# adamjorr/kbbq

Hardware: AMD Instinct MI355X
Metric: recalibrated Gbases/sec (higher is better)
Workload: dtype u64

## Files before the change

### kbbq_amd/csrc/engine.hip

```cpp
#include <hip/hip_runtime.h>

#include <algorithm>
#include <climits>
#include <cstdarg>
#include <cstdio>
#include <cstdlib>
#include <cstring>
#include <map>
#include <mutex>
#include <string>
#include <thread>
#include <vector>

#include "../../include/kbbq_engine.h"
#include "abi_internal.h"
#include "correct.h"
#include "correct_wave.h"
#include "device_common.h"
#include "host_model.h"

using namespace kbbq;

static thread_local char g_err[512] = "";
int kbbq_fail(int code, const char *fmt, ...) {
// ... 27 lines not shown
    FiltDev dev() const {
        FiltDev f;
        f.table = reinterpret_cast<ulonglong2 *>(d_table);
        f.patterns = reinterpret_cast<const ulonglong2 *>(d_patterns);
        f.n_blocks = spec.n_blocks;
        const ModMagic mm = make_mod_magic(spec.n_blocks);
        f.mod_magic = mm.m64;
        f.mod_m32 = mm.m32;
        f.salt0 = spec.salt[0];
        f.salt1 = spec.salt[1];
        return f;
    }
};

struct ProfileSlot {
    std::string name;
    uint64_t launches = 0;
    double ms = 0;
};
struct PendingEvent {
    int slot;
    hipEvent_t a, b;
};

constexpr int kNoOverride = INT_MIN;
struct Options {
    bool no_overlap = false;
    bool no_fastpath = false;
    bool lane_walk = false;
    bool no_pass4_pipeline = false;
    int pass2_side = 2;
    bool tally_general = false;
    bool infer_subset = true;
    bool debug_bucket = false;
    int bucket = -1;
    uint64_t bucket_records = 0;
    uint64_t pass4_piece = 0;
    int scan_blocks = -1;
    int walk_blocks = -1;
    int infer_blocks = 0;
    int subset_edge = kNoOverride;
    int subset_pmask = kNoOverride;
};


enum Scratch {
    S_KMER_PREFIX,
    S_HOST_OUT,
    S_HOST_FLAGS,
    S_DRAW0, S_DRAW1,
    S_TAKE1,
    S_READ_INDEX0, S_READ_INDEX1,
    S_TMASK, S_DIRTY, S_LIST, S_ERR, S_PATCH,
    S_OFFCASE_LIST,
    S_WALK_WORDS,
    S_SIDE1,
    S_COUNT = S_SIDE1 + (S_SIDE1 - S_TMASK),
    S_TAKE0 = S_ERR + (S_SIDE1 - S_TMASK),
};
constexpr int per_side(Scratch name, int side) { return name + side * (S_SIDE1 - S_TMASK); }

struct SideCounters { unsigned long long list_len, queries; };
struct Counters {
    SideCounters side0;
    unsigned long long kmer_total;
    unsigned long long infer_fetched;
// ... 71 lines not shown
    bool cur_h2d_recorded = false;
    bool async_call = false;
    uint64_t last_ticket = 0;
    hipStream_t copy = nullptr;
    uint64_t stats[4] = {0, 0, 0, 0};
    std::vector<ProfileSlot> prof;
    std::vector<PendingEvent> pending;
    uint32_t *d_qcum = nullptr, *d_errthr = nullptr;
    uint32_t qcum_len = 0;
    struct Buckets {
        int mode[2] = {-1, -1};
        bool allocated = false;
        uint64_t capacity = 0;
        void *l1 = nullptr, *l2 = nullptr;
        uint32_t *l1_cnt = nullptr, *l2_cnt = nullptr, *tickets = nullptr;
        unsigned long long *direct = nullptr;
        bool pending[2] = {false, false};
        double pending_est[2] = {0, 0};
        double frac_trusted = 0.75;
        double frac_used = 0.75;
        uint64_t bases_since[2] = {0, 0}, inserted_at_flush[2] = {0, 0};
        uint64_t flushes[2] = {0, 0};
        hipStream_t stream[2] = {nullptr, nullptr};
        hipEvent_t ev_flush = nullptr;
        unsigned long long *h_inserted = nullptr;
        hipEvent_t ev_est = nullptr;
        bool est_pending = false, est_known = false;
        uint64_t est_bases = 0, est_prev = 0, cur_bases = 0;
    } bk;
    hipEvent_t ev_infer = nullptr, ev_take[2] = {nullptr, nullptr};
    bool take_pending[2] = {false, false};
    int take_turn = 0;
    size_t attr_lds_tally = 0, attr_lds_recal = 0;
    std::map<const void *, size_t> attr_lds_correct;
};

namespace {

template <typename T> int scratch_buf(kbbq_engine *e, int name, size_t bytes, T **out) {
    if (e->scratch_bytes[name] < bytes) {
        if (e->scratch[name]) {
            HIP_TRY(hipStreamSynchronize(e->stream));
            HIP_TRY(hipStreamSynchronize(e->stream2));
            HIP_TRY(hipFree(e->scratch[name]));
            e->scratch[name] = nullptr;
            e->scratch_bytes[name] = 0;
        }
        const size_t want = bytes + bytes / 8 + 256;
        HIP_TRY(hipMalloc(&e->scratch[name], want));
        e->scratch_bytes[name] = want;
    }
    *out = static_cast<T *>(e->scratch[name]);
    return KBBQ_OK;
}

int run_after(hipStream_t waiter, hipStream_t signaller, hipEvent_t ev) {
    HIP_TRY(hipEventRecord(ev, signaller));
    HIP_TRY(hipStreamWaitEvent(waiter, ev, 0));
    return KBBQ_OK;
}

std::vector<hipEvent_t *> engine_events(kbbq_engine *e) {
    std::vector<hipEvent_t *> v = {&e->ev_main, &e->ev_draw, &e->ev_ins[0], &e->ev_ins[1], &e->ev_side[0], &e->ev_side[1],
                                   &e->bk.ev_flush, &e->bk.ev_est, &e->ev_infer, &e->ev_take[0], &e->ev_take[1]};
    for (kbbq_engine::StageSlot &s : e->slot) v.insert(v.end(), {&s.h2d, &s.d2h, &s.done[0], &s.done[1]});
    return v;
// ... 483 lines not shown

}


extern "C" {

const char *kbbq_last_error(void) { return g_err; }

int kbbq_engine_create(const kbbq_params *params, kbbq_engine **out) {
    if (!params || !out) return fail(KBBQ_EINVAL, "null argument");
    if (params->k < 1 || params->k > KBBQ_MAX_KMER) return fail(KBBQ_ERANGE, "k must be <= %d and > 0", KBBQ_MAX_KMER);
    if (params->n_rg < 1 || params->n_rg > 65535) return fail(KBBQ_EINVAL, "n_rg must be in 1..65535");
    if (params->max_read_len < 1 || params->max_read_len > KBBQ_MAX_READ_LEN)
        return fail(KBBQ_ERANGE, "max_read_len must be in 1..%d", KBBQ_MAX_READ_LEN);
    int ndev = 0;
    if (hipGetDeviceCount(&ndev) != hipSuccess || ndev == 0) return fail(KBBQ_ENODEV, "no HIP device visible");
    if (params->device < 0 || params->device >= ndev) return fail(KBBQ_ENODEV, "device %d of %d", params->device, ndev);
    DeviceGuard create_guard(params->device);
    HIP_TRY(create_guard.err);
    kbbq_engine *e = new kbbq_engine;
    e->p = *params;
    {
        Options &o = e->opt;
        auto env_set = [](const char *name) { const char *v = getenv(name); return v && *v; };
        auto env_int = [](const char *name, int dflt) { const char *v = getenv(name); return v && *v ? atoi(v) : dflt; };
        const int fl = params->flags;
        o.no_overlap = (fl & KBBQ_F_NO_OVERLAP) || env_set("KBBQ_NO_OVERLAP");
        o.no_fastpath = (fl & KBBQ_F_NO_FASTPATH) || env_set("KBBQ_NO_FASTPATH");
        o.lane_walk = (fl & KBBQ_F_LANE_WALK) || (getenv("KBBQ_CORRECT") && !strcmp(getenv("KBBQ_CORRECT"), "lane"));
        o.no_pass4_pipeline = (fl & KBBQ_F_NO_PASS4_PIPELINE) || env_set("KBBQ_NO_PASS4_PIPELINE");
        o.pass2_side = (fl & KBBQ_F_PASS2_INORDER) ? 0 : env_int("KBBQ_PASS2_SIDE", o.pass2_side);
        o.tally_general = env_set("KBBQ_TALLY_GENERAL");
        o.infer_subset = env_int("KBBQ_INFER_SUBSET", 1) != 0;
        o.debug_bucket = env_set("KBBQ_DEBUG_BUCKET");
        o.bucket = (fl & KBBQ_F_BUCKET_ON) ? 1 : (fl & KBBQ_F_BUCKET_OFF) ? 0 : env_set("KBBQ_BUCKET") ? (env_int("KBBQ_BUCKET", 0) != 0 ? 1 : 0) : -1;
        o.bucket_records = env_u64("KBBQ_BUCKET_RECORDS", 0);
        o.pass4_piece = env_u64("KBBQ_PASS4_PIECE", 0);
        o.scan_blocks = env_int("KBBQ_SCAN_BLOCKS", o.scan_blocks);
        o.walk_blocks = env_int("KBBQ_WALK_BLOCKS", o.walk_blocks);
        o.infer_blocks = env_int("KBBQ_INFER_BLOCKS", o.infer_blocks);
        o.subset_edge = env_int("KBBQ_SUBSET_EDGE", o.subset_edge);
        o.subset_pmask = env_int("KBBQ_SUBSET_PMASK", o.subset_pmask);
    }
    e->K.k = params->k;
    e->K.shift = 2u * (unsigned)(params->k - 1);
    e->K.mask = params->k < 32 ? ((1ULL << (2 * params->k)) - 1) : ~0ULL;
    e->K.nmask_bits = params->k < 32 ? ((1u << params->k) - 1) : 0xFFFFFFFFu;
    const double fprs[2] = {params->fpr_sampled, params->fpr_trusted};
    for (int w = 0; w < 2; ++w) {
        if (!make_filter_spec(params->approx_kmers, fprs[w], params->bloom_seed, e->filt[w].spec)) {
            delete e;
            return fail(KBBQ_EINVAL, "Error: Invalid bloom filter parameters. Adjust parameters and try again.");
        }
    }
    hipError_t he = hipStreamCreateWithFlags(&e->stream, hipStreamNonBlocking);
    if (he == hipSuccess) he = hipStreamCreateWithFlags(&e->stream2, hipStreamNonBlocking);
    if (he == hipSuccess) he = hipStreamCreateWithFlags(&e->copy, hipStreamNonBlocking);
    for (hipEvent_t *ev : engine_events(e))
        if (he == hipSuccess) he = hipEventCreateWithFlags(ev, hipEventDisableTiming);
    if (he == hipSuccess) he = hipHostMalloc((void **)&e->bk.h_inserted, 64, hipHostMallocDefault);
    if (he != hipSuccess) { kbbq_engine_destroy(e); return fail(KBBQ_EIO, "hipStreamCreate: %s", hipGetErrorString(he)); }
#define CREATE_TRY(expr)                                                                           \
    do {                                                                                           \
        hipError_t _e = (expr);                                                                    \
        if (_e != hipSuccess) {                                                                    \
            int code = _e == hipErrorOutOfMemory ? KBBQ_ENOMEM : KBBQ_EIO;                         \
// ... 104 lines not shown
    for (int w = 0; w < 2; ++w) { e->bk.pending[w] = false; e->bk.pending_est[w] = 0; e->bk.bases_since[w] = 0; e->bk.inserted_at_flush[w] = 0; e->bk.flushes[w] = 0; }
    e->thresholds_set = false;
    e->dq_set = false;
    memset(e->stats, 0, sizeof e->stats);
    return sync_engine(e);
}

int kbbq_engine_sync(kbbq_engine *e) {
    ENGINE_DEVICE(e);
    return settle(e);
}

void *kbbq_engine_stream(kbbq_engine *e) { return e ? (void *)e->stream : nullptr; }

int kbbq_engine_dims(kbbq_engine *e, uint64_t *n_rg, uint64_t *n_cycle) {
    if (!e) return fail(KBBQ_EINVAL, "null engine");
    if (n_rg) *n_rg = (uint64_t)e->p.n_rg;
    if (n_cycle) *n_cycle = (uint64_t)e->p.max_read_len;
    return KBBQ_OK;
}

int kbbq_engine_tune(kbbq_engine *e, const char *name, uint64_t value) {
    if (!e || !name) return fail(KBBQ_EINVAL, "null argument");
    if (!strcmp(name, "bucket_records")) {
        if (e->bk.allocated) return fail(KBBQ_ESTATE, "the record buffers are allocated already");
        e->opt.bucket_records = value;
    } else if (!strcmp(name, "pass4_piece")) {
        e->opt.pass4_piece = value;
    } else if (!strcmp(name, "scan_blocks") || !strcmp(name, "walk_blocks") || !strcmp(name, "infer_blocks")) {
        if (value > 17) return fail(KBBQ_EINVAL, "%s: 0 (as many as fit) to 16 workgroups per CU, 17 = default", name);
        (name[0] == 's' ? e->opt.scan_blocks : name[0] == 'w' ? e->opt.walk_blocks : e->opt.infer_blocks) = value == 17 ? (name[0] == 'i' ? 0 : -1) : (int)value;
    } else if (!strcmp(name, "infer_subset")) {
        e->opt.infer_subset = value != 0;
    } else if (!strcmp(name, "pass2_side") || !strcmp(name, "no_overlap")) {
        ENGINE_DEVICE(e);
        int rc = settle(e);
        if (rc) return rc;
        if (name[0] == 'p' && value > 2) return fail(KBBQ_EINVAL, "pass2_side: 0, 1 or 2");
        if (name[0] == 'p') e->opt.pass2_side = (int)value; else e->opt.no_overlap = value != 0;
        e->bk.stream[0] = e->bk.stream[1] = nullptr;
    } else {
        return fail(KBBQ_EINVAL, "unknown knob '%s'", name);
    }
    return KBBQ_OK;
}

int kbbq_filter_info_get(kbbq_engine *e, int which, kbbq_filter_info *out) {
    ENGINE_DEVICE(e);
    if (!out || which < 0 || which > 1) return fail(KBBQ_EINVAL, "bad argument");
    int rc = settle(e);
    if (rc) return rc;
    const FilterSpec &s = e->filt[which].spec;
    memset(out, 0, sizeof *out);
    out->bits = s.bits;
    out->bits_unblocked = s.bits_unblocked;
    out->n_blocks = s.n_blocks;
    out->table_bytes = e->filt[which].table_bytes();
    out->random_seed = s.random_seed;
    out->n_hash = s.n_hash;
    out->n_salt = s.n_salt;
    for (uint32_t i = 0; i < s.n_salt; ++i) out->salt[i] = s.salt[i];
    HIP_TRY(hipMemcpy(&out->inserted, e->filt[which].d_inserted, 8, hipMemcpyDeviceToHost));
    return KBBQ_OK;
}

void *kbbq_filter_device_table(kbbq_engine *e, int which) {
// ... 817 lines not shown
    hipLaunchKernelGGL(k_read_index, dim3((unsigned)((R.n_reads + 255) / 256)), dim3(256), 0, stream, R.offsets, R.n_reads, d);
    HIP_TRY(hipGetLastError());
    *index = d;
    return KBBQ_OK;
}

static int run_tally(kbbq_engine *e, const Pass3 &c, const ReadsDev &R, const uint32_t *err_bits, const uint32_t *patch, int max_len) {
    const hipStream_t stream = c.stream;
    HistDev H;
    H.cycle = e->d_hist;
    H.dinuc = e->d_hist + e->hist_cycle_words;
    H.n_rg = e->p.n_rg;
    H.n_cycle = e->p.max_read_len;
    const int n_rg = R.rg ? e->p.n_rg : 1;
    const int ccap = std::min(((max_len + 31) / 32) * 32, 192);
    if (!e->qpresent_known) {
        hipLaunchKernelGGL(k_qpresence, dim3(1024), dim3(256), 0, stream, R.qual, R.n_bases, e->d_qpresent);
        HIP_TRY(hipGetLastError());
        HIP_TRY(hipMemcpyAsync(e->qpresent, e->d_qpresent, 32, hipMemcpyDeviceToHost, stream));
        HIP_TRY(hipStreamSynchronize(stream));
    }
    const int n_windows = (max_len + ccap - 1) / ccap;
    const bool direct_cycles = n_windows > kTallyMaxWindows;
    const size_t per_slot = (direct_cycles ? 0 : (size_t)8 * ccap) + 128;
    TallyPlan P;
    plan_tally_slots(P, e->qpresent, (int)((152 * 1024 - 512) / per_slot), n_rg);
    P.direct_cycles = direct_cycles ? 1 : 0;
    const size_t per_rg = (size_t)P.n_slots * per_slot;
    const size_t budget = (size_t)n_rg * per_rg <= 70 * 1024 ? 70 * 1024 : 140 * 1024;
    const int per_launch = (int)std::max<size_t>(1, std::min<size_t>((size_t)n_rg, budget / per_rg));
    const size_t lds = (size_t)per_launch * per_rg + 4 + 256 + 4;
    if (lds > e->attr_lds_tally) {
        HIP_TRY(hipFuncSetAttribute((const void *)k_tally, hipFuncAttributeMaxDynamicSharedMemorySize, (int)lds));
        HIP_TRY(hipFuncSetAttribute((const void *)k_tally_uniform<true>, hipFuncAttributeMaxDynamicSharedMemorySize, (int)lds));
        HIP_TRY(hipFuncSetAttribute((const void *)k_tally_uniform<false>, hipFuncAttributeMaxDynamicSharedMemorySize, (int)lds));
        e->attr_lds_tally = lds;
    }
    const uint64_t groups = (R.n_bases + 15) / 16;
    const int blocks = (int)std::min<uint64_t>((groups + 1023) / 1024, lds <= 76 * 1024 ? 512 : 256);
    const int vec_ok = ((uintptr_t)R.qual & 15) == 0;
    const uint32_t *read_index;
    int rc = build_read_index(e, R, c.stream_no, stream, &read_index);
    if (rc) return rc;
    const uint32_t *present = nullptr;
    if (n_rg > per_launch) {
        uint32_t *pr = e->d_rg_present[c.stream_no];
        HIP_TRY(hipMemsetAsync(pr, 0, (((size_t)e->p.n_rg + 31) / 32) * 4, stream));
        hipLaunchKernelGGL(k_rg_presence, dim3((unsigned)((R.n_reads + 255) / 256)), dim3(256), 0, stream, R.rg, R.n_reads, (uint32_t)e->p.n_rg, pr);
        present = pr;
    }
    if (!e->opt.tally_general && !R.offsets && n_rg == 1 && n_windows == 1 && R.read_len >= 16 && (int)R.read_len <= ccap && R.n_bases < (1ULL << 32) && vec_ok &&
        e->p.n_rg == 1) {
        const unsigned long long inv_len = ~0ULL / R.read_len + 1;
        Timed t(e, "k_tally", stream);
        if (P.identity) hipLaunchKernelGGL(k_tally_uniform<false>, dim3(blocks), dim3(1024), lds, stream, R, H, err_bits, patch, ccap, 6, inv_len, P);
        else hipLaunchKernelGGL(k_tally_uniform<true>, dim3(blocks), dim3(1024), lds, stream, R, H, err_bits, patch, ccap, 6, inv_len, P);
        HIP_TRY(hipGetLastError());
        return KBBQ_OK;
    }
    Timed t(e, "k_tally", stream);
    for (int g = 0; g < n_rg; g += per_launch)
        for (int w = 0; w < (direct_cycles ? 1 : n_windows); ++w) {
            P.rg_base = g;
            P.n_rgs = std::min(per_launch, n_rg - g);
            P.cbase = w * ccap;
            hipLaunchKernelGGL(k_tally, dim3(blocks), dim3(1024), lds, stream, R, H, err_bits, patch, ccap, 6, vec_ok, P, present, read_index);
        }
    HIP_TRY(hipGetLastError());
    return KBBQ_OK;
}

int kbbq_errors_batch(kbbq_engine *e, const kbbq_reads *reads, uint64_t *errors_out) {
    ENGINE_DEVICE(e);
    { int frc = bucket_flush_all(e); if (frc) return frc; }
    if (!reads) return fail(KBBQ_EINVAL, "null argument");
    const bool own_err = !(errors_out && reads->on_device);
    const bool overlap = own_err && !(errors_out && !reads->on_device) && !e->opt.no_overlap;
    int side = 0, rc;
    if (overlap) {
        side = e->side_turn;
        e->side_turn ^= 1;
        if (e->side_busy[side]) HIP_TRY(hipStreamWaitEvent(e->stream, e->ev_side[side], 0));
    } else {
        if ((rc = sync_engine(e))) return rc;
    }
    HostBatchDone host_done(e, reads);
    ReadsDev R; int max_len;
    if ((rc = device_view(e, reads, &R, &max_len))) return rc;
    const bool long_reads = max_len > kStagedMax;
// ... 210 lines not shown
static int recalibrate_impl(kbbq_engine *e, const kbbq_reads *reads, uint8_t *qual_out, bool out_on_host) {
    ENGINE_DEVICE(e);
    if (!qual_out || !reads) return fail(KBBQ_EINVAL, "null argument");
    if (!e->dq_set) return fail(KBBQ_ESTATE, "no delta-Q tables yet");
    HostBatchDone host_done(e, reads);
    ReadsDev R; int max_len;
    const bool no_pipe = e->opt.no_pass4_pipeline || e->opt.no_overlap;
    const uint64_t piece_env = e->opt.pass4_piece;
    const uint64_t piece = piece_env ? ((piece_env + 63) >> 6) << 6 : std::max<uint64_t>(1ull << 23, ((reads->n_bases / 4 + 65535) >> 16) << 16);
    const bool pipelined = !reads->on_device && out_on_host && !no_pipe && reads->n_bases >= 2 * piece;
    DeferredCopy dc;
    const bool deferred_out = e->async_call && !reads->on_device && out_on_host;
    SlotOutput so;
    so.bytes = reads->n_bases + 16;
    int rc = device_view(e, reads, &R, &max_len, true, pipelined ? &dc : nullptr, deferred_out ? &so : nullptr);
    if (rc) return rc;
    uint8_t *d_out = qual_out;
    if (deferred_out) {
        d_out = (uint8_t *)so.dev;
    } else if (out_on_host) {
        if ((rc = scratch_buf(e, S_HOST_OUT, R.n_bases + 16, &d_out))) return rc;
    }
    DqDev D;
    D.base = e->d_dq_base; D.cycle = e->d_dq_cycle; D.dinuc = e->d_dq_dinuc;
    D.qslot = e->d_dq_qslot;
    D.n_rg = e->p.n_rg; D.n_cycle = e->p.max_read_len; D.n_slots = e->dq_slots;
    const uint32_t *read_index;
    if ((rc = build_read_index(e, R, 0, e->stream, &read_index))) return rc;
    const int per_rg = (D.n_slots * (4 * D.n_cycle + 16) + KBBQ_NQ * 2 + 3) & ~3;
    const int budget = per_rg + 256 <= 64 * 1024 ? 64 * 1024 - 256 : 152 * 1024 - 256;
    const int lds_rgs = D.n_slots > 255 ? 0 : std::max(0, std::min(D.n_rg, budget / per_rg));
    const size_t lds = 256 + (size_t)lds_rgs * per_rg;
    if (lds > e->attr_lds_recal) {
        HIP_TRY(hipFuncSetAttribute((const void *)k_recalibrate, hipFuncAttributeMaxDynamicSharedMemorySize, (int)lds));
        e->attr_lds_recal = lds;
    }
    const int vec_ok = (((uintptr_t)R.qual | (uintptr_t)d_out) & 15) == 0;
    auto launch = [&](uint64_t base0, uint64_t base1) -> int {
        Timed t(e, "k_recalibrate");
        const uint64_t lanes = (base1 - base0 + 15) / 16;
        const unsigned blocks = (unsigned)std::min<uint64_t>((lanes + 1023) / 1024, lds > 76 * 1024 ? 256 : 256 * 2);
        hipLaunchKernelGGL(k_recalibrate, dim3(blocks), dim3(1024), lds, e->stream,
                           R, D, d_out, 6, vec_ok, lds_rgs, read_index, base0, base1);
        HIP_TRY(hipGetLastError());
        return KBBQ_OK;
    };
    if (pipelined) {
        const uint64_t nb = R.n_bases;
        struct SideDone {
            hipStream_t st;
            bool wait;
            ~SideDone() { if (wait) (void)hipStreamSynchronize(st); }
        } side_done{e->stream2, !deferred_out};
        for (uint64_t b0 = 0; b0 < nb; b0 += piece) {
            const uint64_t b1 = std::min(nb, b0 + piece);
            const uint64_t w0 = b0 / 32, w1 = b1 == nb ? nb / 32 + 1 : b1 / 32, m0 = b0 / 64, m1 = b1 == nb ? nb / 64 + 1 : b1 / 64;
            HIP_TRY(hipMemcpyAsync(dc.d_bases + w0 * 8, reads->bases + w0, (w1 - w0) * 8, hipMemcpyHostToDevice, e->copy));
            HIP_TRY(hipMemcpyAsync(dc.d_nmask + m0 * 8, reads->nmask + m0, (m1 - m0) * 8, hipMemcpyHostToDevice, e->copy));
            HIP_TRY(hipMemcpyAsync(dc.d_qual + b0, reads->qual + b0, b1 - b0, hipMemcpyHostToDevice, e->copy));
            if ((rc = run_after(e->stream, e->copy, dc.slot->h2d))) return rc;
            if ((rc = launch(b0, b1))) return rc;
            if ((rc = run_after(e->stream2, e->stream, e->ev_main))) return rc;
            HIP_TRY(hipMemcpyAsync(qual_out + b0, d_out + b0, b1 - b0, hipMemcpyDeviceToHost, e->stream2));
        }
        if (deferred_out) {
            HIP_TRY(hipEventRecord(so.slot->d2h, e->stream2));
            so.slot->d2h_pending = true;
            e->cur_slot_side = true;
            return KBBQ_OK;
        }
        HIP_TRY(hipStreamSynchronize(e->stream2));
        return KBBQ_OK;
    }
    if ((rc = launch(0, R.n_bases))) return rc;
    if (out_on_host) {
        HIP_TRY(hipMemcpyAsync(qual_out, d_out, R.n_bases, hipMemcpyDeviceToHost, e->stream));
// ... 233 lines not shown
```

### kbbq_amd/csrc/kernels.h

```cpp
#pragma once
#include <hip/hip_runtime.h>

#include "../../include/kbbq_engine.h"
#include "correct.h"
#include "correct_wave.h"
#include "device_common.h"

using namespace kbbq;


constexpr int DRAWS_PER_LANE = 4096;

__constant__ uint64_t c_jump[64][4];

__device__ __forceinline__ uint64_t xo_next(uint64_t (&s)[4]) {
    uint64_t x = s[1] * 5;
    x = (x << 7) | (x >> 57);
    x *= 9;
    const uint64_t t = s[1] << 17;
    s[2] ^= s[0];
    s[3] ^= s[1];
    s[1] ^= s[2];
    s[0] ^= s[3];
    s[2] ^= t;
// ... 906 lines not shown
                uint32_t *t = lds + lr * per_rg;
                const int rg = P.rg_base + lr;
                for (int w = threadIdx.x; w < cyc_words; w += blockDim.x) {
                    const uint32_t v = t[w], ve = t[cyc_words + w];
                    if (!v) continue;
                    t[w] = 0;
                    t[cyc_words + w] = 0;
                    for (int h = 0; h < 2; ++h) {
                        const uint32_t cnt = (v >> (16 * h)) & 0xFFFFu, cne = (ve >> (16 * h)) & 0xFFFFu;
                        if (!cnt) continue;
                        const int idx = 2 * w + h;
                        const int slot = idx % ccap, rest = idx / ccap;
                        const int q = P.qof[rest % ns], s = rest / ns;
                        const int c = cbase + (slot % (ccap >> 4)) * 16 + slot / (ccap >> 4);
                        if (c < H.n_cycle) {
                            atomicAdd(&H.cycle[cyc_index(H, rg, q, s, c) + 1], (unsigned long long)cnt);
                            if (cne) atomicAdd(&H.cycle[cyc_index(H, rg, q, s, c)], (unsigned long long)cne);
                        }
                    }
                }
                for (int w = threadIdx.x; w < ns * 16; w += blockDim.x) {
                    const uint32_t v = t[2 * cyc_words + w], ve = t[2 * cyc_words + ns * 16 + w];
                    const uint64_t cell = ((uint64_t)rg * KBBQ_NQ + P.qof[w >> 4]) * 16 + (w & 15);
                    if (v) { t[2 * cyc_words + w] = 0; atomicAdd(&H.dinuc[cell * 2 + 1], (unsigned long long)v); }
                    if (ve) { t[2 * cyc_words + ns * 16 + w] = 0; atomicAdd(&H.dinuc[cell * 2], (unsigned long long)ve); }
                }
            }
            if (threadIdx.x == 0) *l_reads = 0;
            __syncthreads();
        }
    }
}

template <bool MAP>
__global__ void __launch_bounds__(1024) k_tally_uniform(ReadsDev R, HistDev H, const uint32_t *err_bits, const uint32_t *patch,
                                                         int ccap, int minscore, unsigned long long inv_len, TallyPlan P) {
    extern __shared__ uint32_t lds[];
    const int ns = P.n_slots;
    const int L = (int)R.read_len;
    const int cyc_words = (2 * ccap * ns + 1) / 2, cstep = ccap >> 4;
    uint32_t *t_err = lds + cyc_words, *t_di = lds + 2 * cyc_words, *t_die = t_di + ns * 16;
    const int lds_words = 2 * cyc_words + 2 * ns * 16;
    uint8_t *l_qslot = reinterpret_cast<uint8_t *>(lds + lds_words);
    for (int i = threadIdx.x; i < lds_words; i += blockDim.x) lds[i] = 0;
    if (MAP && threadIdx.x < 256) l_qslot[threadIdx.x] = P.qslot[threadIdx.x];
    __syncthreads();
    auto count = [&](int second, int q, int cyc, int er, bool dinuc_ok, int d) {
        const int sl = MAP ? (int)l_qslot[q] : q;
        if (MAP ? sl != 255 : sl < ns) {
            const int idx = (second * ns + sl) * ccap + (cyc & 15) * cstep + (cyc >> 4);
            const uint32_t one = 1u << (16 * (idx & 1));
            atomicAdd(&lds[idx >> 1], one);
            if (er) atomicAdd(&t_err[idx >> 1], one);
            if (dinuc_ok) {
                atomicAdd(&t_di[sl * 16 + d], 1u);
                if (er) atomicAdd(&t_die[sl * 16 + d], 1u);
            }
        } else {
            atomicAdd(&H.cycle[cyc_index(H, 0, q, second, cyc) + 1], 1ULL);
            if (er) atomicAdd(&H.cycle[cyc_index(H, 0, q, second, cyc)], 1ULL);
            if (dinuc_ok) {
                atomicAdd(&H.dinuc[((uint64_t)q * 16 + d) * 2 + 1], 1ULL);
                if (er) atomicAdd(&H.dinuc[((uint64_t)q * 16 + d) * 2], 1ULL);
            }
        }
    };
    auto flush = [&]() {
        for (int w = threadIdx.x; w < cyc_words; w += blockDim.x) {
            const uint32_t v = lds[w], ve = t_err[w];
            if (!v) continue;
            lds[w] = 0;
            t_err[w] = 0;
            for (int h = 0; h < 2; ++h) {
                const uint32_t cnt = (v >> (16 * h)) & 0xFFFFu, cne = (ve >> (16 * h)) & 0xFFFFu;
                if (!cnt) continue;
                const int idx = 2 * w + h;
                const int slot = idx % ccap, rest = idx / ccap;
                const int q = MAP ? (int)P.qof[rest % ns] : rest % ns, sec = rest / ns;
                const int c = (slot % cstep) * 16 + slot / cstep;
                if (c < H.n_cycle) {
                    atomicAdd(&H.cycle[cyc_index(H, 0, q, sec, c) + 1], (unsigned long long)cnt);
                    if (cne) atomicAdd(&H.cycle[cyc_index(H, 0, q, sec, c)], (unsigned long long)cne);
                }
            }
        }
        for (int w = threadIdx.x; w < ns * 16; w += blockDim.x) {
            const uint32_t v = t_di[w], ve = t_die[w];
            const uint64_t cell = (uint64_t)(MAP ? (int)P.qof[w >> 4] : (w >> 4)) * 16 + (w & 15);
            if (v) { t_di[w] = 0; atomicAdd(&H.dinuc[cell * 2 + 1], (unsigned long long)v); }
            if (ve) { t_die[w] = 0; atomicAdd(&H.dinuc[cell * 2], (unsigned long long)ve); }
        }
    };
    const uint64_t n_groups = (R.n_bases + 15) / 16;
    const uint64_t stride = (uint64_t)gridDim.x * blockDim.x;
    const uint64_t iters = (n_groups + stride - 1) / stride;
    const uint64_t flush_every = max((uint64_t)1, (uint64_t)40000 / ((uint64_t)16384 / (uint64_t)L + 2));
    for (uint64_t it = 0; it < iters; ++it) {
        const uint64_t g0 = (it * stride + (uint64_t)blockIdx.x * blockDim.x + threadIdx.x) * 16;
        if (g0 + 16 <= R.n_bases) {
            const uint32_t r = (uint32_t)__umul64hi((unsigned long long)g0, inv_len);
            const int c0 = (int)(g0 - (uint64_t)r * (uint64_t)L);
            const int bpos = L - c0 < 16 ? L - c0 : 16;
            const uint4 qv4 = *reinterpret_cast<const uint4 *>(R.qual + g0);
            uint8_t qv[16];
            memcpy(qv, &qv4, 16);
            const uint32_t bw = (uint32_t)(R.bases[g0 >> 5] >> ((g0 & 31) * 2));
            const uint32_t nw = (uint32_t)(R.nmask[g0 >> 6] >> (g0 & 63)) & 0xFFFFu;
            const uint32_t ew = (err_bits[g0 >> 5] >> (g0 & 31)) & 0xFFFFu;
            int prev_b = 0, prev_n = 1;
            if (g0 > 0) {
                const uint64_t gp = g0 - 1;
                prev_b = (int)((R.bases[gp >> 5] >> ((gp & 31) * 2)) & 3);
                prev_n = (int)((R.nmask[gp >> 6] >> (gp & 63)) & 1);
            }
            const bool two = bpos < 16;
            const bool mine1 = !R.rg || R.rg[r] == 0, mine2 = !two || !R.rg || R.rg[r + 1] == 0;
            const int sec1 = R.flags ? (R.flags[r] & 1) : 0;
            const int sec2 = two && R.flags ? (R.flags[r + 1] & 1) : 0;
            const uint32_t pt1 = patch ? patch[r] : 0u, pt2 = two && patch ? patch[r + 1] : 0u;
            const int pp1 = (pt1 >> 31) ? patch_at(pt1) : -2, pp2 = (pt2 >> 31) ? patch_at(pt2) : -2;
            if (pp1 >= 0 && pp1 == c0 - 1) { prev_b = (int)(pt1 & 3); prev_n = 0; }
#pragma unroll
            for (int i = 0; i < 16; ++i) {
                const bool in2 = i >= bpos;
                const int cyc = c0 + i - (in2 ? L : 0);
                int b = (int)((bw >> (2 * i)) & 3), nn = (int)((nw >> i) & 1);
                if (cyc == (in2 ? pp2 : pp1)) { b = (int)((in2 ? pt2 : pt1) & 3); nn = 0; }
                const int q = qv[i];
                if (in2 ? mine2 : mine1)
                    count(in2 ? sec2 : sec1, q, cyc, (int)((ew >> i) & 1u), cyc >= 1 && q >= minscore && !(nn | prev_n), (prev_b << 2) | b);
                prev_b = b;
                prev_n = nn;
            }
        } else if (g0 < R.n_bases) {
            for (uint64_t g = g0; g < R.n_bases; ++g) {
                const uint64_t r = g / (uint64_t)L;
                const int cyc = (int)(g - r * (uint64_t)L);
                const uint32_t pt = patch ? patch[r] : 0u;
                const int pp = (pt >> 31) ? patch_at(pt) : -2;
                auto base_at = [&](uint64_t x, int cx, int &bb, int &nb) {
                    bb = (int)((R.bases[x >> 5] >> ((x & 31) * 2)) & 3);
                    nb = (int)((R.nmask[x >> 6] >> (x & 63)) & 1);
                    if (cx == pp) { bb = (int)(pt & 3); nb = 0; }
                };
                int b, nn, pb = 0, pn = 1;
                base_at(g, cyc, b, nn);
                if (cyc >= 1) base_at(g - 1, cyc - 1, pb, pn);
                const int q = R.qual[g];
                const int er = (int)((err_bits[g >> 5] >> (g & 31)) & 1u);
                if (!R.rg || R.rg[r] == 0)
                    count(R.flags ? (R.flags[r] & 1) : 0, q, cyc, er, cyc >= 1 && q >= minscore && !(nn | pn), (pb << 2) | b);
            }
        }
        if ((it + 1) % flush_every == 0 || it + 1 == iters) {
            __syncthreads();
            flush();
            __syncthreads();
        }
    }
}

__global__ void __launch_bounds__(256) k_qpresence(const uint8_t *qual, uint64_t n_bases, uint32_t *qpresent) {
    __shared__ uint32_t qseen[8];
    if (threadIdx.x < 8) qseen[threadIdx.x] = 0;
    __syncthreads();
    for (uint64_t i = (uint64_t)blockIdx.x * blockDim.x + threadIdx.x; i < n_bases; i += (uint64_t)gridDim.x * blockDim.x)
        qseen_note(qseen, qual[i]);
    __syncthreads();
    if (threadIdx.x < 8 && qseen[threadIdx.x]) atomicOr(&qpresent[threadIdx.x], qseen[threadIdx.x]);
}

struct DqDev {
    const int16_t *base;
    const int8_t *cycle;
    const int8_t *dinuc;
    const uint8_t *qslot;
    int n_rg, n_cycle, n_slots;
};

__global__ void __launch_bounds__(1024) k_recalibrate(ReadsDev R, DqDev D, uint8_t *out, int minqual, int vec_ok, int lds_rgs,
                                                       const uint32_t *read_index, uint64_t base0, uint64_t base1) {
    extern __shared__ uint8_t l_tab[];
    uint8_t *l_qslot = l_tab;
    const int ns = D.n_slots;
    const int cyc_cells = ns * 2 * D.n_cycle, di_bytes = ns * 16, base_bytes = KBBQ_NQ * 2;
    const int cyc_bytes = 2 * cyc_cells;
    const int per_rg = (cyc_bytes + di_bytes + base_bytes + 3) & ~3;
    uint8_t *l_rg = l_tab + 256;
    if (threadIdx.x < 256) l_qslot[threadIdx.x] = D.qslot[threadIdx.x];
    __syncthreads();
    for (int i = threadIdx.x; i < lds_rgs * KBBQ_NQ; i += blockDim.x) {
        const int rg = i / KBBQ_NQ, q = i % KBBQ_NQ;
        reinterpret_cast<int16_t *>(l_rg + (size_t)rg * per_rg + cyc_bytes + di_bytes)[q] = D.base[rg * KBBQ_NQ + q];
        const int sl = l_qslot[q];
        if (sl != 255) {
            int16_t *tc = reinterpret_cast<int16_t *>(l_rg + (size_t)rg * per_rg) + sl * 2 * D.n_cycle;
            const int8_t *src = D.cycle + ((size_t)rg * KBBQ_NQ + q) * 2 * D.n_cycle;
            for (int c = 0; c < 2 * D.n_cycle; ++c) tc[c] = (int16_t)(D.base[rg * KBBQ_NQ + q] + src[c]);
            for (int x = 0; x < 16; ++x) l_rg[(size_t)rg * per_rg + cyc_bytes + sl * 16 + x] = (uint8_t)D.dinuc[((size_t)rg * KBBQ_NQ + q) * 16 + x];
        }
    }
    __syncthreads();
    for (uint64_t g0 = base0 + ((uint64_t)blockIdx.x * blockDim.x + threadIdx.x) * 16; g0 < base1;
         g0 += (uint64_t)gridDim.x * blockDim.x * 16) {
    uint64_t r, start, end;
    if (R.offsets) {
        find_read(R, read_index, g0, r, start, end);
    } else {
        r = g0 / R.read_len;
        start = r * R.read_len;
        end = start + R.read_len;
    }
    const int n = (int)min((uint64_t)16, R.n_bases - g0);
    uint8_t qv[16];
    if (n == 16 && vec_ok) {
        const uint4 v = *reinterpret_cast<const uint4 *>(R.qual + g0);
        memcpy(qv, &v, 16);
    } else {
        for (int i = 0; i < 16; ++i) qv[i] = i < n ? R.qual[g0 + i] : 0;
    }
    const uint32_t bw = (uint32_t)(R.bases[g0 >> 5] >> ((g0 & 31) * 2));
    const uint32_t nw = (uint32_t)(R.nmask[g0 >> 6] >> (g0 & 63)) & 0xFFFFu;
    int prev_b = 0, prev_n = 1;
    if (g0 > 0) {
        const uint64_t gp = g0 - 1;
        prev_b = (int)((R.bases[gp >> 5] >> ((gp & 31) * 2)) & 3);
        prev_n = (int)((R.nmask[gp >> 6] >> (gp & 63)) & 1);
    }
    int rg = R.rg ? (int)R.rg[r] : 0;
    int second = R.flags ? (R.flags[r] & 1) : 0;
    uint8_t res[16];
    const int bpos = end - g0 < 16 ? (int)(end - g0) : 16;
    int rg2 = rg, second2 = second;
    uint64_t end2 = end;
    if (bpos < 16 && r + 1 < R.n_reads) {
        rg2 = R.rg ? (int)R.rg[r + 1] : 0;
        second2 = R.flags ? (R.flags[r + 1] & 1) : 0;
        end2 = R.offsets ? R.offsets[r + 2] : end + R.read_len;
    }
    const int c0 = (int)(g0 - start);
    const bool plain = n == 16 && rg < lds_rgs && rg2 < lds_rgs && (bpos == 16 || (r + 1 < R.n_reads && end2 >= g0 + 16)) &&
                       c0 + bpos <= D.n_cycle && 16 - bpos <= D.n_cycle;
    if (plain) {
        const int16_t *ta = reinterpret_cast<const int16_t *>(l_rg + rg * per_rg) + second * D.n_cycle + c0;
        const int16_t *tb = reinterpret_cast<const int16_t *>(l_rg + rg2 * per_rg) + second2 * D.n_cycle - bpos;
        const int8_t *da = reinterpret_cast<const int8_t *>(l_rg + rg * per_rg + cyc_bytes);
        const int8_t *db = reinterpret_cast<const int8_t *>(l_rg + rg2 * per_rg + cyc_bytes);
        const int16_t *ba = reinterpret_cast<const int16_t *>(l_rg + rg * per_rg + cyc_bytes + di_bytes);
        const int16_t *bb = reinterpret_cast<const int16_t *>(l_rg + rg2 * per_rg + cyc_bytes + di_bytes);
        const int qstride = 2 * D.n_cycle;
#pragma unroll
        for (int i = 0; i < 16; ++i) {
            const bool in2 = i >= bpos;
            const int b = (int)((bw >> (2 * i)) & 3), nn = (int)((nw >> i) & 1);
            const int q = qv[i];
            int v = q;
            if (q >= minqual) {
                const int sl = l_qslot[q];
                if (sl != 255) {
                    v = (in2 ? tb : ta)[sl * qstride + i];
                    const bool first = in2 ? i == bpos : c0 + i == 0;
                    if (!first && !(nn | prev_n)) v += (in2 ? db : da)[sl * 16 + ((prev_b << 2) | b)];
                } else {
                    v = (in2 ? bb : ba)[q];
                }
            }
            res[i] = (uint8_t)(v < 0 ? 0 : (v > KBBQ_MAXQ ? KBBQ_MAXQ : v));
            prev_b = b;
            prev_n = nn;
        }
    } else {
#pragma unroll
    for (int i = 0; i < 16; ++i) {
        const uint64_t g = g0 + i;
        if (i < n) {
            while (g >= end) {
// ... 122 lines not shown
```

Baseline: 24.14.

## Add branch-free straight-line paths for the tally and recalibrate kernels

Adds templated straight-line variants of k_tally_uniform and k_recalibrate, both enabled by default. The tally packs count and error into one LDS word with an XOR-swizzled cycle index and takes a 16-base fast path that needs no per-base branching. Recalibrate replaces the read division with a multiply-high and computes all 16 outputs with unconditional LDS loads and masks instead of branches. Launch occupancy is now derived from a HIP occupancy query. The risk is more register pressure and extra LDS loads, and the packed 16-bit counters could overflow if many counts land in one cell between flushes.

```diff
diff --git a/kbbq_amd/csrc/engine.hip b/kbbq_amd/csrc/engine.hip
--- a/kbbq_amd/csrc/engine.hip
+++ b/kbbq_amd/csrc/engine.hip
@@ -83,6 +83,7 @@
     int pass2_side = 2;
     bool tally_general = false;
     bool infer_subset = true;
+    int straight_line = 3;
     bool debug_bucket = false;
     int bucket = -1;
     uint64_t bucket_records = 0;
@@ -220,6 +221,7 @@
     bool take_pending[2] = {false, false};
     int take_turn = 0;
     size_t attr_lds_tally = 0, attr_lds_recal = 0;
+    size_t recal_sl_lds = ~(size_t)0; int recal_sl_per_cu = 1;
     std::map<const void *, size_t> attr_lds_correct;
 };
 
@@ -769,6 +771,7 @@
         o.pass2_side = (fl & KBBQ_F_PASS2_INORDER) ? 0 : env_int("KBBQ_PASS2_SIDE", o.pass2_side);
         o.tally_general = env_set("KBBQ_TALLY_GENERAL");
         o.infer_subset = env_int("KBBQ_INFER_SUBSET", 1) != 0;
+        o.straight_line = env_int("KBBQ_STRAIGHT_LINE", o.straight_line) & 3;
         o.debug_bucket = env_set("KBBQ_DEBUG_BUCKET");
         o.bucket = (fl & KBBQ_F_BUCKET_ON) ? 1 : (fl & KBBQ_F_BUCKET_OFF) ? 0 : env_set("KBBQ_BUCKET") ? (env_int("KBBQ_BUCKET", 0) != 0 ? 1 : 0) : -1;
         o.bucket_records = env_u64("KBBQ_BUCKET_RECORDS", 0);
@@ -939,6 +942,9 @@
         (name[0] == 's' ? e->opt.scan_blocks : name[0] == 'w' ? e->opt.walk_blocks : e->opt.infer_blocks) = value == 17 ? (name[0] == 'i' ? 0 : -1) : (int)value;
     } else if (!strcmp(name, "infer_subset")) {
         e->opt.infer_subset = value != 0;
+    } else if (!strcmp(name, "straight_line")) {
+        if (value > 3) return fail(KBBQ_EINVAL, "straight_line: bit 0 the tally, bit 1 the apply (0 to 3)");
+        e->opt.straight_line = (int)value;
     } else if (!strcmp(name, "pass2_side") || !strcmp(name, "no_overlap")) {
         ENGINE_DEVICE(e);
         int rc = settle(e);
@@ -1822,8 +1828,10 @@
     const size_t lds = (size_t)per_launch * per_rg + 4 + 256 + 4;
     if (lds > e->attr_lds_tally) {
         HIP_TRY(hipFuncSetAttribute((const void *)k_tally, hipFuncAttributeMaxDynamicSharedMemorySize, (int)lds));
-        HIP_TRY(hipFuncSetAttribute((const void *)k_tally_uniform<true>, hipFuncAttributeMaxDynamicSharedMemorySize, (int)lds));
-        HIP_TRY(hipFuncSetAttribute((const void *)k_tally_uniform<false>, hipFuncAttributeMaxDynamicSharedMemorySize, (int)lds));
+        HIP_TRY(hipFuncSetAttribute((const void *)k_tally_uniform<true, false>, hipFuncAttributeMaxDynamicSharedMemorySize, (int)lds));
+        HIP_TRY(hipFuncSetAttribute((const void *)k_tally_uniform<false, false>, hipFuncAttributeMaxDynamicSharedMemorySize, (int)lds));
+        HIP_TRY(hipFuncSetAttribute((const void *)k_tally_uniform<true, true>, hipFuncAttributeMaxDynamicSharedMemorySize, (int)lds));
+        HIP_TRY(hipFuncSetAttribute((const void *)k_tally_uniform<false, true>, hipFuncAttributeMaxDynamicSharedMemorySize, (int)lds));
         e->attr_lds_tally = lds;
     }
     const uint64_t groups = (R.n_bases + 15) / 16;
@@ -1843,8 +1851,9 @@
         e->p.n_rg == 1) {
         const unsigned long long inv_len = ~0ULL / R.read_len + 1;
         Timed t(e, "k_tally", stream);
-        if (P.identity) hipLaunchKernelGGL(k_tally_uniform<false>, dim3(blocks), dim3(1024), lds, stream, R, H, err_bits, patch, ccap, 6, inv_len, P);
-        else hipLaunchKernelGGL(k_tally_uniform<true>, dim3(blocks), dim3(1024), lds, stream, R, H, err_bits, patch, ccap, 6, inv_len, P);
+        auto kernel = e->opt.straight_line & 1 ? (P.identity ? k_tally_uniform<false, true> : k_tally_uniform<true, true>)
+                                               : (P.identity ? k_tally_uniform<false, false> : k_tally_uniform<true, false>);
+        hipLaunchKernelGGL(kernel, dim3(blocks), dim3(1024), lds, stream, R, H, err_bits, patch, ccap, 6, inv_len, P);
         HIP_TRY(hipGetLastError());
         return KBBQ_OK;
     }
@@ -2121,16 +2130,27 @@
     const int lds_rgs = D.n_slots > 255 ? 0 : std::max(0, std::min(D.n_rg, budget / per_rg));
     const size_t lds = 256 + (size_t)lds_rgs * per_rg;
     if (lds > e->attr_lds_recal) {
-        HIP_TRY(hipFuncSetAttribute((const void *)k_recalibrate, hipFuncAttributeMaxDynamicSharedMemorySize, (int)lds));
+        HIP_TRY(hipFuncSetAttribute((const void *)k_recalibrate<false>, hipFuncAttributeMaxDynamicSharedMemorySize, (int)lds));
+        HIP_TRY(hipFuncSetAttribute((const void *)k_recalibrate<true>, hipFuncAttributeMaxDynamicSharedMemorySize, (int)lds));
         e->attr_lds_recal = lds;
     }
     const int vec_ok = (((uintptr_t)R.qual | (uintptr_t)d_out) & 15) == 0;
+    const unsigned long long inv_len = !R.offsets && R.read_len >= 2 && R.n_bases < (1ULL << 32) ? ~0ULL / R.read_len + 1 : 0;
+    const bool straight = (e->opt.straight_line & 2) != 0;
+    auto kernel = straight ? k_recalibrate<true> : k_recalibrate<false>;
+    if (straight && e->recal_sl_lds != lds) {
+        int n = 1;
+        HIP_TRY(hipOccupancyMaxActiveBlocksPerMultiprocessor(&n, k_recalibrate<true>, 1024, lds));
+        e->recal_sl_per_cu = std::max(1, std::min(n, 2));
+        e->recal_sl_lds = lds;
+    }
+    const unsigned per_cu = lds > 76 * 1024 ? 1 : straight ? (unsigned)e->recal_sl_per_cu : 2;
     auto launch = [&](uint64_t base0, uint64_t base1) -> int {
         Timed t(e, "k_recalibrate");
         const uint64_t lanes = (base1 - base0 + 15) / 16;
-        const unsigned blocks = (unsigned)std::min<uint64_t>((lanes + 1023) / 1024, lds > 76 * 1024 ? 256 : 256 * 2);
-        hipLaunchKernelGGL(k_recalibrate, dim3(blocks), dim3(1024), lds, e->stream,
-                           R, D, d_out, 6, vec_ok, lds_rgs, read_index, base0, base1);
+        const unsigned blocks = (unsigned)std::min<uint64_t>((lanes + 1023) / 1024, 256 * per_cu);
+        hipLaunchKernelGGL(kernel, dim3(blocks), dim3(1024), lds, e->stream,
+                           R, D, d_out, 6, vec_ok, lds_rgs, read_index, base0, base1, inv_len);
         HIP_TRY(hipGetLastError());
         return KBBQ_OK;
     };
diff --git a/kbbq_amd/csrc/kernels.h b/kbbq_amd/csrc/kernels.h
--- a/kbbq_amd/csrc/kernels.h
+++ b/kbbq_amd/csrc/kernels.h
@@ -962,7 +962,7 @@
     }
 }
 
-template <bool MAP>
+template <bool MAP, bool SL>
 __global__ void __launch_bounds__(1024) k_tally_uniform(ReadsDev R, HistDev H, const uint32_t *err_bits, const uint32_t *patch,
                                                          int ccap, int minscore, unsigned long long inv_len, TallyPlan P) {
     extern __shared__ uint32_t lds[];
@@ -970,6 +970,7 @@
     const int L = (int)R.read_len;
     const int cyc_words = (2 * ccap * ns + 1) / 2, cstep = ccap >> 4;
     uint32_t *t_err = lds + cyc_words, *t_di = lds + 2 * cyc_words, *t_die = t_di + ns * 16;
+    unsigned long long *t_di2 = reinterpret_cast<unsigned long long *>(t_di);
     const int lds_words = 2 * cyc_words + 2 * ns * 16;
     uint8_t *l_qslot = reinterpret_cast<uint8_t *>(lds + lds_words);
     for (int i = threadIdx.x; i < lds_words; i += blockDim.x) lds[i] = 0;
@@ -978,6 +979,11 @@
     auto count = [&](int second, int q, int cyc, int er, bool dinuc_ok, int d) {
         const int sl = MAP ? (int)l_qslot[q] : q;
         if (MAP ? sl != 255 : sl < ns) {
+            if (SL) {
+                atomicAdd(&lds[(second * ns + sl) * ccap + (cyc ^ ((cyc >> 4) & 15))], 1u | ((uint32_t)er << 16));
+                if (dinuc_ok) atomicAdd(&t_di2[sl * 16 + (((d & 3) << 2) | (d >> 2))], 1ULL | ((unsigned long long)er << 32));
+                return;
+            }
             const int idx = (second * ns + sl) * ccap + (cyc & 15) * cstep + (cyc >> 4);
             const uint32_t one = 1u << (16 * (idx & 1));
             atomicAdd(&lds[idx >> 1], one);
@@ -996,6 +1002,29 @@
         }
     };
     auto flush = [&]() {
+        if (SL) {
+            for (int w = threadIdx.x; w < 2 * ns * ccap; w += blockDim.x) {
+                const uint32_t v = lds[w];
+                if (!v) continue;
+                lds[w] = 0;
+                const int pos = w % ccap, rest = w / ccap;
+                const int q = MAP ? (int)P.qof[rest % ns] : rest % ns, sec = rest / ns;
+                const int c = pos ^ ((pos >> 4) & 15);
+                if (c < H.n_cycle) {
+                    atomicAdd(&H.cycle[cyc_index(H, 0, q, sec, c) + 1], (unsigned long long)(v & 0xFFFFu));
+                    if (v >> 16) atomicAdd(&H.cycle[cyc_index(H, 0, q, sec, c)], (unsigned long long)(v >> 16));
+                }
+            }
+            for (int w = threadIdx.x; w < ns * 16; w += blockDim.x) {
+                const unsigned long long v = t_di2[w];
+                if (!v) continue;
+                t_di2[w] = 0;
+                const uint64_t cell = (uint64_t)(MAP ? (int)P.qof[w >> 4] : (w >> 4)) * 16 + (((w & 3) << 2) | ((w >> 2) & 3));
+                atomicAdd(&H.dinuc[cell * 2 + 1], v & 0xFFFFFFFFULL);
+                if (v >> 32) atomicAdd(&H.dinuc[cell * 2], v >> 32);
+            }
+            return;
+        }
         for (int w = threadIdx.x; w < cyc_words; w += blockDim.x) {
             const uint32_t v = lds[w], ve = t_err[w];
             if (!v) continue;
@@ -1050,6 +1079,59 @@
             const uint32_t pt1 = patch ? patch[r] : 0u, pt2 = two && patch ? patch[r + 1] : 0u;
             const int pp1 = (pt1 >> 31) ? patch_at(pt1) : -2, pp2 = (pt2 >> 31) ? patch_at(pt2) : -2;
             if (pp1 >= 0 && pp1 == c0 - 1) { prev_b = (int)(pt1 & 3); prev_n = 0; }
+            uint32_t slv[16];
+            bool fast = false;
+            if (SL) {
+                uint32_t top[16];
+#pragma unroll
+                for (int i = 0; i < 16; ++i) top[i] = slv[i] = MAP ? (uint32_t)l_qslot[qv[i]] : (uint32_t)qv[i];
+#pragma unroll
+                for (int w = 8; w; w >>= 1)
+#pragma unroll
+                    for (int i = 0; i < w; ++i) top[i] = max(top[i], top[i + w]);
+                fast = (MAP ? top[0] != 255u : top[0] < (uint32_t)ns) & mine1 & mine2;
+            }
+            if (SL && fast) {
+                const uint32_t i1 = (uint32_t)(pp1 - c0), i2 = (uint32_t)(pp2 + bpos);
+                const bool h1 = i1 < (uint32_t)bpos, h2 = (uint32_t)pp2 < (uint32_t)(16 - bpos);
+                const uint32_t s1 = h1 ? i1 : 0u, s2 = h2 ? i2 : 0u;
+                uint32_t bwp = bw, nwp = nw;
+                bwp = h1 ? (bwp & ~(3u << (2 * s1))) | ((pt1 & 3u) << (2 * s1)) : bwp;
+                nwp = h1 ? nwp & ~(1u << s1) : nwp;
+                bwp = h2 ? (bwp & ~(3u << (2 * s2))) | ((pt2 & 3u) << (2 * s2)) : bwp;
+                nwp = h2 ? nwp & ~(1u << s2) : nwp;
+                const uint32_t n17 = (nwp << 1) | (uint32_t)prev_n;
+                const uint32_t okm = ~(n17 | (n17 >> 1) | (c0 == 0 ? 1u : 0u) | (two ? 1u << bpos : 0u));
+                const uint64_t win = ((uint64_t)bwp << 2) | (uint64_t)prev_b;
+                const uint32_t secrow = (uint32_t)(ns * ccap) << 16;
+                const uint32_t p1 = (sec1 ? secrow : 0u) | (uint32_t)c0;
+                const uint32_t p2 = (sec2 ? secrow : 0u) | (uint32_t)(512 - bpos);
+#pragma unroll
+                for (int i = 0; i < 16; ++i) {
+                    const uint32_t t = (i >= bpos ? p2 : p1) + (uint32_t)i;
+                    const uint32_t pos = (t & 255u) ^ ((t >> 4) & 15u);
+                    const uint32_t er = (ew >> i) & 1u;
+                    atomicAdd(&lds[__umul24(slv[i], (uint32_t)ccap) + (t >> 16) + pos], 1u | (er << 16));
+                    if (((okm >> i) & 1u) & (uint32_t)((int)qv[i] >= minscore))
+                        atomicAdd(&t_di2[slv[i] * 16u + (uint32_t)((win >> (2 * i)) & 15u)], 1ULL | ((unsigned long long)er << 32));
+                }
+            } else if (SL) {
+                const uint64_t qlo = (uint64_t)qv4.x | ((uint64_t)qv4.y << 32), qhi = (uint64_t)qv4.z | ((uint64_t)qv4.w << 32);
+#pragma unroll 1
+                for (int i = 0; i < 16; ++i) {
+                    const bool in2 = i >= bpos;
+                    const int cyc = c0 + i - (in2 ? L : 0);
+                    int b = (int)((bw >> (2 * i)) & 3), nn = (int)((nw >> i) & 1);
+                    const bool pat = cyc == (in2 ? pp2 : pp1);
+                    b = pat ? (int)((in2 ? pt2 : pt1) & 3) : b;
+                    nn = pat ? 0 : nn;
+                    const int q = (int)(((i & 8 ? qhi : qlo) >> ((i & 7) * 8)) & 255);
+                    if (in2 ? mine2 : mine1)
+                        count(in2 ? sec2 : sec1, q, cyc, (int)((ew >> i) & 1u), cyc >= 1 && q >= minscore && !(nn | prev_n), (prev_b << 2) | b);
+                    prev_b = b;
+                    prev_n = nn;
+                }
+            } else {
 #pragma unroll
             for (int i = 0; i < 16; ++i) {
                 const bool in2 = i >= bpos;
@@ -1061,6 +1143,7 @@
                     count(in2 ? sec2 : sec1, q, cyc, (int)((ew >> i) & 1u), cyc >= 1 && q >= minscore && !(nn | prev_n), (prev_b << 2) | b);
                 prev_b = b;
                 prev_n = nn;
+            }
             }
         } else if (g0 < R.n_bases) {
             for (uint64_t g = g0; g < R.n_bases; ++g) {
@@ -1108,8 +1191,10 @@
     int n_rg, n_cycle, n_slots;
 };
 
+template <bool SL>
 __global__ void __launch_bounds__(1024) k_recalibrate(ReadsDev R, DqDev D, uint8_t *out, int minqual, int vec_ok, int lds_rgs,
-                                                       const uint32_t *read_index, uint64_t base0, uint64_t base1) {
+                                                       const uint32_t *read_index, uint64_t base0, uint64_t base1,
+                                                       unsigned long long inv_len) {
     extern __shared__ uint8_t l_tab[];
     uint8_t *l_qslot = l_tab;
     const int ns = D.n_slots;
@@ -1136,6 +1221,10 @@
     uint64_t r, start, end;
     if (R.offsets) {
         find_read(R, read_index, g0, r, start, end);
+    } else if (SL && inv_len) {
+        r = __umul64hi((unsigned long long)g0, inv_len);
+        start = r * R.read_len;
+        end = start + R.read_len;
     } else {
         r = g0 / R.read_len;
         start = r * R.read_len;
@@ -1171,7 +1260,40 @@
     const int c0 = (int)(g0 - start);
     const bool plain = n == 16 && rg < lds_rgs && rg2 < lds_rgs && (bpos == 16 || (r + 1 < R.n_reads && end2 >= g0 + 16)) &&
                        c0 + bpos <= D.n_cycle && 16 - bpos <= D.n_cycle;
-    if (plain) {
+    if (SL && plain && ns > 0) {
+        uint32_t sl[16];
+#pragma unroll
+        for (int i = 0; i < 16; ++i) sl[i] = l_qslot[qv[i]];
+        const uint32_t xa = (uint32_t)(rg * per_rg + (second * D.n_cycle + c0) * 2);
+        const uint32_t xb = (uint32_t)(rg2 * per_rg + (second2 * D.n_cycle - bpos) * 2);
+        const uint32_t ra = (uint32_t)(rg * per_rg + cyc_bytes), rb = (uint32_t)(rg2 * per_rg + cyc_bytes);
+        const uint32_t qbytes = (uint32_t)(4 * D.n_cycle);
+        const uint32_t n17 = (nw << 1) | (uint32_t)prev_n;
+        const uint32_t okm = ~(n17 | (n17 >> 1) | (c0 == 0 ? 1u : 0u) | (bpos < 16 ? 1u << bpos : 0u));
+        const uint64_t win = ((uint64_t)bw << 2) | (uint64_t)prev_b;
+        const uint32_t w0 = (uint32_t)win, w1 = (uint32_t)(win >> 2);
+        const uint32_t we = ((w0 & 0x33333333u) << 2) | ((w0 >> 2) & 0x33333333u);
+        const uint32_t wo = ((w1 & 0x33333333u) << 2) | ((w1 >> 2) & 0x33333333u);
+        int vc[16], vd[16], vb[16];
+#pragma unroll
+        for (int i = 0; i < 16; ++i) {
+            const bool in2 = i >= bpos;
+            const uint32_t slc = min(sl[i], (uint32_t)(ns - 1));
+            const uint32_t d = ((i & 1 ? wo : we) >> (4 * (i >> 1))) & 15u;
+            const uint32_t tr = in2 ? rb : ra;
+            vc[i] = *reinterpret_cast<const int16_t *>(l_rg + (in2 ? xb : xa) + __umul24(slc, qbytes) + 2 * i);
+            vd[i] = *reinterpret_cast<const int8_t *>(l_rg + tr + slc * 16u + d);
+            vb[i] = *reinterpret_cast<const int16_t *>(l_rg + tr + (uint32_t)di_bytes + 2u * qv[i]);
+        }
+#pragma unroll
+        for (int i = 0; i < 16; ++i) {
+            const int q = qv[i];
+            int v = vc[i] + (vd[i] & ((int)(okm << (31 - i)) >> 31));
+            v = sl[i] == 255u ? vb[i] : v;
+            v = q >= minqual ? v : q;
+            res[i] = (uint8_t)(v < 0 ? 0 : (v > KBBQ_MAXQ ? KBBQ_MAXQ : v));
+        }
+    } else if (plain) {
         const int16_t *ta = reinterpret_cast<const int16_t *>(l_rg + rg * per_rg) + second * D.n_cycle + c0;
         const int16_t *tb = reinterpret_cast<const int16_t *>(l_rg + rg2 * per_rg) + second2 * D.n_cycle - bpos;
         const int8_t *da = reinterpret_cast<const int8_t *>(l_rg + rg * per_rg + cyc_bytes);
```

New measurement: 23.65. 0.98x the previous value.
